# Isaac-McPadden/Farkle_II

Hardware: AMD Instinct MI355X
Metric: simulated games/sec (whole node) at k=2, fixed strategy-grid size (higher is better)
Workload: dtype int32; 1 GPU; BASELINE configs[1]: k=2, 64-strategy grid, 10^7 games per GPU per step, root_seed 42, counts-only tallies; k=2, root_seed=42, parallelism=shuffle-range split x1, device=AMD Radeon Graphics, arch=gfx950:sramecc+:xnack-, compute_units=256, clock_mhz=2400

## Files before the change

### farkle_ii_amd/csrc/farkle_hip.hip

```cpp
#include "fk_kernels.h"
#include "fk_shard_writer.h"
#include "fk_perm_wave.h"
#include "fk_row_columns_seats.h"
#include "fk_matchups.h"
#include "fk_game_stats.h"
#include "fk_bootstrap.h"

#include <dlfcn.h>
#include <rccl/rccl.h>
#include <unistd.h>

#include <algorithm>
#include <atomic>
#include <chrono>
#include <memory>
#include <mutex>
#include <sys/mman.h>
#include <unordered_map>
#include <thread>
#include <cstdarg>
#include <cstdio>
#include <cstring>
#include <string>
#include <vector>
// ... 16 lines not shown
    }
};

struct ChunkSet {
    DevBuf perm, draws, state, inc, seat_idx, order, classes, misc, pools;
    DevBuf blocks, game_block, game_row;
    hipEvent_t ready = nullptr;
    hipEvent_t ev[4] = {nullptr, nullptr, nullptr, nullptr};
    bool prepared = false;
    bool side = false;
    ChunkDesc desc;
    SeedArgs sa{};
};

struct GameStatsReq {
    int64_t rare_target;
    uint32_t rounds_bins, margin_bins;
    int64_t *s_counts, *s_rounds, *s_runner, *s_spread;
    int64_t *g_counts, *g_rounds, *g_runner;
    int64_t spill_capacity;
    int64_t *spill_count;
    int32_t *spill;
};

struct fk_ctx {
    int device = 0;
    hipStream_t stream = nullptr;
    hipStream_t prep_stream = nullptr;
    ChunkSet sets[2];
    int cur = 0;
    uint64_t table_epoch = 0;
    bool hint_valid = false;
    uint64_t hint_begin = 0, hint_end = 0;
    int32_t hint_state = 0, pipeline = 1;
    hipDeviceProp_t prop{};
    std::string err;
    fk_timing timing{};
    std::string play_instance;
    hipEvent_t ev[8] = {nullptr, nullptr, nullptr, nullptr, nullptr, nullptr, nullptr, nullptr};
    int32_t *err_host = nullptr;
    hipEvent_t main_idle = nullptr;
    struct PendingTimer {
        float *acc;
        hipEvent_t a, b;
    };
    std::vector<PendingTimer> pending;
// ... 18 lines not shown
    int32_t batch_threshold = 0;
    int32_t use_lds_tally = -1;
    int32_t block = 0;
    int32_t hc = -1;
    int32_t hc_waves = 5;
    int32_t hc_block = 256;
    int32_t hc_tables = 1;
    int32_t hc_inc_regs = 1;
    int32_t hc_cl = -1;
    DevBuf lds_tables;
    DevBuf cold;
    int32_t clock_stamps = 0;
    DevBuf clk;
    int clk_grid = 0;
    DevBuf lag_v, lag_out, lag_lags, lag_edge, lag_tmp;
    DevBuf m_ids, m_dig, m_seat, m_rnd;
    DevBuf mr[36];
    uint64_t matchup_sort_mask = ~0ull;
    DevBuf g_rec, g_out;
    int64_t game_stats_window = 0;
    const GameStatsReq *gstats = nullptr;
    DevBuf boot[8];
    int64_t bootstrap_block = 0;
    bool ran_hc = false;
    int32_t perm_split = -1;
    int32_t columns_by_seat = -1;
    int32_t perm_draw_wave = -1;
    void *comm = nullptr;
    int comm_rank = 0, comm_world = 1;
    bool comm_async = false;
    bool comm_lost = false;
    bool comm_timeout_set = false;
    int32_t comm_timeout_ms = 120000;
    DevBuf comm_buf;
    DevBuf rows_alt;
    const int32_t *columns_ids = nullptr;
    uint32_t *want_shuffle_seeds = nullptr, *want_game_seeds = nullptr;
    DevBuf ids;
    hipStream_t copy_stream = nullptr;
    hipEvent_t ev_rows[2] = {nullptr, nullptr}, ev_copy[2] = {nullptr, nullptr};
    int32_t rows_async = 0;
    hipEvent_t ev_call_copy[FK_ROWS_EVENTS] = {};
    uint32_t rows_calls = 0;
    uint8_t *mail = nullptr;
    size_t mail_cap = 0, mail_used = 0;
    struct Letter { void *dst; size_t off, bytes; };
    std::vector<Letter> letters;
    int32_t last_rows_event = -1;
    int64_t rows_chunk_games = 4000000;
// ... 144 lines not shown
    ss_begin(p, 2u , purpose, (uint32_t)root_seed, (uint32_t)(root_seed >> 32));
    ss_absorb64(p, k);
    return p;
}

struct LaunchPlan {
    int block = 0, grid = 0, cus = 1;
    mutable int launched_grid = 0;
    mutable const char *instance = nullptr;
    size_t lds = 0;
    bool lds_tally = false;
    bool lean = false;
    bool gs = false;
    bool blk = false;
    bool hc = false;
    bool hc_lt = false;
    int hc_ki = 0;
    bool hc_cl = false;
    int wpe = 4;
    uint32_t mixed_flags = 0xff00u;
};

constexpr size_t LDS_LIMIT = 160 * 1024;

size_t play_lds_bytes(int32_t k, int block, bool lean, bool gs, bool lds_tally, int32_t S, bool blocks_mode = false) {
    const size_t per_lane = (size_t)(lean ? LEAN_DW : NF) * 4 * (size_t)(gs ? 1 : k) + (blocks_mode ? 4 : 0);
    return per_lane * (size_t)block + (lds_tally ? (size_t)S * LT_COLS * 8 : 0);
}

LaunchPlan plan_play(const fk_ctx *c, int32_t k, int64_t S, bool single_batch, int32_t target_score, bool blocks_mode = false) {
    LaunchPlan best;
    const bool lean_ok = ceil_div50(target_score) <= LEAN_MAX_TARGET50;
    if (blocks_mode) {
        if (!lean_ok) return best;
        best.block = 768;
        best.lean = true;
        best.blk = true;
        best.wpe = 6;
        best.lds = play_lds_bytes(2, 768, true, false, false, 0, true);
        const int per_cu = c->blocks_per_cu > 0 ? std::min(2, c->blocks_per_cu) : 2;
        best.grid = c->prop.multiProcessorCount * per_cu;
        best.cus = c->prop.multiProcessorCount;
        return best;
    }
    const bool want_tally = single_batch && !blocks_mode && (c->use_lds_tally != 0) && S <= 4096;
    int best_lanes = -1;
// ... 297 lines not shown
            const uint32_t n_words = (uint32_t)(bytes / 4);
            hipLaunchKernelGGL(fk_mail_kernel, dim3(std::min<uint32_t>((n_words + 255u) / 256u, 1024u)), dim3(256), 0, c->stream,
                               static_cast<const uint32_t *>(src), reinterpret_cast<uint32_t *>(c->mail + off), n_words);
            HIPCHK(c, hipGetLastError());
            c->letters.push_back({dst, off, bytes});
            c->mail_used = off + bytes;
            return FK_OK;
        }
    }
    HIPCHK(c, hipMemcpyAsync(dst, src, bytes, hipMemcpyDeviceToHost, c->stream));
    return FK_OK;
}

void reserve_mail(fk_ctx *c, size_t bytes) {
    if (!c->letters.empty() || bytes <= c->mail_cap || !rows_dma_pending(c)) return;
    if (c->mail) (void)hipHostFree(c->mail);
    c->mail = nullptr;
    c->mail_cap = 0;
    const size_t cap = std::max<size_t>((size_t)4 << 20, (bytes + ((size_t)1 << 20)) & ~(((size_t)1 << 20) - 1));
    if (hipHostMalloc(reinterpret_cast<void **>(&c->mail), cap, hipHostMallocDefault) == hipSuccess) c->mail_cap = cap;
    else (void)hipGetLastError();
}

void deliver_mail(fk_ctx *c) {
    for (const auto &l : c->letters) std::memcpy(l.dst, c->mail + l.off, l.bytes);
    c->letters.clear();
    c->mail_used = 0;
}

int check_device_error(fk_ctx *c, const int32_t *d_err, int64_t game_base, const char *what) {
    int32_t h[2] = {0, 0};
    const int rc = post_d2h(c, h, d_err, sizeof(h));
    if (rc) return rc;
    HIPCHK(c, hipStreamSynchronize(c->stream));
    deliver_mail(c);
    return report_device_error(c, h, game_base, what);
}

int upload_overrides(fk_ctx *c, std::vector<DevOverride> &dov) {
    if (dov.empty()) return FK_OK;
    std::sort(dov.begin(), dov.end(), [](const DevOverride &x, const DevOverride &y) { return x.game < y.game; });
    int rc = ensure(c, c->ov, dov.size() * sizeof(DevOverride));
    if (rc) return rc;
    HIPCHK(c, hipMemcpyAsync(c->ov.p, dov.data(), dov.size() * sizeof(DevOverride), hipMemcpyHostToDevice, c->stream));
    HIPCHK(c, hipStreamSynchronize(c->stream));
    return FK_OK;
}


int seed_stage(fk_ctx *c, int si, hipStream_t st, SeedArgs &sa, bool full_state, bool timed) {
    ChunkSet &cs = c->sets[si];
    sa.state_dw = full_state ? STATE_DW : 4u;
    int rc = ensure(c, cs.state, (size_t)sa.n_games * sa.k * sa.state_dw * 4);
    if (rc) return rc;
    rc = ensure(c, cs.inc, (size_t)sa.n_games * sa.k * 16);
    if (rc) return rc;
    rc = ensure(c, cs.misc, 512);
    if (rc) return rc;
    HIPCHK(c, hipMemsetAsync(cs.misc.p, 0, 512, st));
    sa.state = static_cast<uint32_t *>(cs.state.p);
    sa.inc = static_cast<uint4 *>(cs.inc.p);
    sa.seat_idx = nullptr;
    if (sa.perm_T && !full_state) {
        rc = ensure(c, cs.seat_idx, (size_t)sa.n_games * sa.k * 2);
        if (rc) return rc;
        sa.seat_idx = static_cast<uint16_t *>(cs.seat_idx.p);
    }
    if (sa.blocks) {
        hipLaunchKernelGGL(fk_block_map_kernel, dim3((sa.n_games + 255u) / 256u), dim3(256), 0, st, sa.blocks, sa.n_blocks,
                           sa.n_games, const_cast<uint32_t *>(sa.game_block), const_cast<uint32_t *>(sa.game_row));
        HIPCHK(c, hipGetLastError());
    }
    if ((sa.perm_T || sa.blocks) && c->longest_first) {
        rc = ensure(c, cs.order, (size_t)sa.n_games * 4);
        if (rc) return rc;
        sa.sched = static_cast<uint32_t *>(cs.order.p);
        sa.sched_ctr = reinterpret_cast<uint32_t *>(static_cast<uint8_t *>(cs.misc.p) + 256);
        rc = ensure(c, cs.classes, 64);
        if (rc) return rc;
        HIPCHK(c, hipMemsetAsync(cs.classes.p, 0, 64, st));
        sa.class_ctr = static_cast<const uint32_t *>(cs.classes.p);
        sa.patience = static_cast<const uint8_t *>(c->slow.p);
    } else {
        sa.sched = nullptr;
    }
    if (timed) (void)hipEventRecord(cs.ev[2], st);
    sa.pools = nullptr;
    if (!sa.coords) {
        const uint32_t n = sa.blocks ? sa.n_blocks : (sa.gps ? (sa.n_games + sa.gps - 1u) / sa.gps : 1u);
        rc = ensure(c, cs.pools, (size_t)n * 16);
        if (rc) return rc;
        sa.pools = static_cast<const uint4 *>(cs.pools.p);
        hipLaunchKernelGGL(fk_pool_kernel, dim3((n + 255u) / 256u), dim3(256), 0, st, sa.prefix, sa.shuffle0, sa.pair, sa.order, sa.blocks, n,
                           static_cast<uint4 *>(cs.pools.p));
    }
    if (sa.sched)
        hipLaunchKernelGGL(fk_class_count_kernel, dim3(std::min<uint32_t>((sa.n_games + SEED_BLOCK - 1u) / SEED_BLOCK, 1024u)), dim3(SEED_BLOCK), 0,
                           st, sa.perm_T, sa.perm_slots, sa.S, sa.k, sa.n_sh, sa.n_games, sa.patience,
                           sa.blocks ? sa.game_row : nullptr, static_cast<uint32_t *>(cs.classes.p));
    hipLaunchKernelGGL(fk_seed_kernel, dim3((sa.n_games + SEED_BLOCK - 1u) / SEED_BLOCK), dim3(SEED_BLOCK), 0, st, sa);
    if (timed) (void)hipEventRecord(cs.ev[3], st);
    HIPCHK(c, hipGetLastError());
    return FK_OK;
}

size_t game_workspace_bytes(int32_t k, bool full_state, bool recs, bool rows) {
    return (size_t)k * ((full_state ? STATE_DW * 4 : 18) + 16) + 8 + (recs ? REC_DW * 4 + 4 : 0) +
           (rows ? sizeof(fk_row_hdr) + sizeof(fk_seat) * (size_t)k : 0);
}

int launch_play_stage(fk_ctx *c, const SeedArgs &sa, PlayArgs &pa, const LaunchPlan &plan, bool want_state, bool want_rec0, bool want_recs) {
    ChunkSet &cs = CSET(c);
    int rc;
    if (want_rec0) {
        rc = ensure(c, c->rec0, (size_t)sa.n_games * 4);
        if (rc) return rc;
    }
    if (want_recs) {
        rc = ensure(c, c->recs, (size_t)sa.n_games * REC_DW * 4);
// ... 79 lines not shown

int finish_play(fk_ctx *c, const PlayArgs &pa, int64_t game_base, const char *what) {
    const int rc_dev = check_device_error(c, pa.err, game_base, what);
    const int rc = finish_timers(c);
    return rc_dev ? rc_dev : rc;
}

int run_chunk(fk_ctx *c, const SeedArgs &sa_in, PlayArgs pa, const LaunchPlan &plan, bool want_state, bool want_rec0, bool want_recs,
              int64_t game_base, const char *what) {
    SeedArgs sa = sa_in;
    ChunkSet &cs = CSET(c);
    cs.prepared = false;
    cs.side = false;
    HIPCHK(c, hipStreamWaitEvent(c->stream, cs.ready, 0));
    (void)hipEventRecord(cs.ev[0], c->stream);
    (void)hipEventRecord(cs.ev[1], c->stream);
    int rc = seed_stage(c, c->cur, c->stream, sa, plan.gs || want_state, true);
    if (rc) return rc;
    rc = launch_play_stage(c, sa, pa, plan, want_state, want_rec0, want_recs);
    if (rc) return rc;
    return finish_play(c, pa, game_base, what);
}

int prep_tournament_chunk(fk_ctx *c, int si, hipStream_t st_seed, const ChunkDesc &d, SeedArgs &sa) {
    ChunkSet &cs = c->sets[si];
    cs.prepared = false;
    hipStream_t st = c->stream;
    HIPCHK(c, hipStreamWaitEvent(st, cs.ready, 0));
    const int32_t S = (int32_t)d.S;
    const uint32_t n_sh = d.n_sh, slots = d.slots, gps = d.S / d.k;
    const uint32_t perm_blocks = (n_sh + slots - 1u) / slots;
    const SeedPool perm_prefix = seed_prefix(101u , d.root, (uint64_t)d.k);
    int rc = ensure(c, cs.perm, (size_t)perm_blocks * S * slots * 2);
    if (rc) return rc;
    (void)hipEventRecord(cs.ev[0], st);
    {
        const size_t perm_lds = (size_t)slots * S * 2;
        static int perm_configured = -1;
        if (perm_configured != c->device) {
            HIPCHK(c, hipFuncSetAttribute(reinterpret_cast<const void *>(&fk_perm_kernel),
                                          hipFuncAttributeMaxDynamicSharedMemorySize, (int)LDS_LIMIT));
            HIPCHK(c, hipFuncSetAttribute(reinterpret_cast<const void *>(&fk_perm_apply_kernel),
                                          hipFuncAttributeMaxDynamicSharedMemorySize, (int)LDS_LIMIT));
            HIPCHK(c, hipFuncSetAttribute(reinterpret_cast<const void *>(&fk_perm_parallel_kernel),
                                          hipFuncAttributeMaxDynamicSharedMemorySize, (int)(LDS_LIMIT - 1024)));
            perm_configured = c->device;
        }
        const bool split = c->perm_split >= 1 || (c->perm_split < 0 && S >= 1024 && n_sh >= 256);
        const size_t pp_lds = (size_t)S * 14;
        const bool parallel = split && c->perm_split != 1 && pp_lds <= LDS_LIMIT - 1024;
        const bool wave_draw = c->perm_draw_wave == 1 || (c->perm_draw_wave < 0 && n_sh <= WAVE_DRAW_MAX_SH);
        if (parallel) {
            const uint32_t groups = ((uint32_t)S - 1u + 7u) / 8u, row_u4 = groups + 1u;
            rc = ensure(c, cs.draws, (size_t)n_sh * row_u4 * 16);
            if (rc) return rc;
            if (wave_draw)
                hipLaunchKernelGGL(fk_perm_draw_wave_kernel, dim3((n_sh + WAVE_DRAW_BLOCK / 64 - 1u) / (WAVE_DRAW_BLOCK / 64)), dim3(WAVE_DRAW_BLOCK), 0, st,
                                   perm_prefix, d.sh0, n_sh, (uint32_t)S, 1u, row_u4, static_cast<uint4 *>(cs.draws.p));
            else
                hipLaunchKernelGGL(fk_perm_draw_kernel, dim3((n_sh + DRAW_BLOCK - 1u) / DRAW_BLOCK), dim3(DRAW_BLOCK), 0, st,
                                   perm_prefix, d.sh0, n_sh, (uint32_t)S, 1u, row_u4, static_cast<uint4 *>(cs.draws.p));
            hipLaunchKernelGGL(fk_perm_parallel_kernel, dim3(n_sh), dim3(PP_BLOCK), pp_lds, st,
                               static_cast<uint4 *>(cs.draws.p), row_u4, n_sh, (uint32_t)S);
            hipLaunchKernelGGL(fk_perm_block_kernel, dim3(((uint32_t)S + 255u) / 256u, perm_blocks), dim3(256), 0, st,
                               static_cast<const uint16_t *>(cs.draws.p), row_u4 * 8u, n_sh, (uint32_t)S, slots,
                               static_cast<uint16_t *>(cs.perm.p));
        } else if (split) {
            const uint32_t n_sh_pad = (n_sh + 63u) & ~63u, groups = ((uint32_t)S - 1u + 7u) / 8u;
            rc = ensure(c, cs.draws, (size_t)groups * n_sh_pad * 16);
            if (rc) return rc;
            if (wave_draw)
                hipLaunchKernelGGL(fk_perm_draw_wave_kernel, dim3((n_sh + WAVE_DRAW_BLOCK / 64 - 1u) / (WAVE_DRAW_BLOCK / 64)), dim3(WAVE_DRAW_BLOCK), 0, st,
                                   perm_prefix, d.sh0, n_sh, (uint32_t)S, n_sh_pad, 1u, static_cast<uint4 *>(cs.draws.p));
            else
                hipLaunchKernelGGL(fk_perm_draw_kernel, dim3((n_sh + DRAW_BLOCK - 1u) / DRAW_BLOCK), dim3(DRAW_BLOCK), 0, st,
                                   perm_prefix, d.sh0, n_sh, (uint32_t)S, n_sh_pad, 1u, static_cast<uint4 *>(cs.draws.p));
            hipLaunchKernelGGL(fk_perm_apply_kernel, dim3(perm_blocks), dim3(PERM_BLOCK), perm_lds, st,
                               static_cast<const uint4 *>(cs.draws.p), n_sh_pad, n_sh, (uint32_t)S, slots,
                               static_cast<uint16_t *>(cs.perm.p));
        } else {
            hipLaunchKernelGGL(fk_perm_kernel, dim3(perm_blocks), dim3(PERM_BLOCK), perm_lds, st,
                               perm_prefix, d.sh0, n_sh, (uint32_t)S, slots, static_cast<uint16_t *>(cs.perm.p));
        }
        HIPCHK(c, hipGetLastError());
    }
    (void)hipEventRecord(cs.ev[1], st);
    sa = SeedArgs{};
    sa.prefix = seed_prefix(103u , d.root, (uint64_t)d.k);
    sa.coords = nullptr;
    sa.shuffle0 = d.sh0;
    sa.gps = gps;
    sa.k = d.k;
    sa.n_games = n_sh * gps;
    sa.perm_T = static_cast<const uint16_t *>(cs.perm.p);
    sa.perm_slots = slots;
    sa.S = d.S;
    sa.n_sh = n_sh;
    if (st_seed != st) {
        HIPCHK(c, hipStreamWaitEvent(st_seed, cs.ev[1], 0));
        HIPCHK(c, hipStreamWaitEvent(st_seed, c->main_idle, 0));
    }
    rc = seed_stage(c, si, st_seed, sa, d.state_dw == STATE_DW, true);
    if (rc) return rc;
    HIPCHK(c, hipEventRecord(cs.ready, st_seed));
    cs.desc = d;
    cs.prepared = true;
    cs.side = (st_seed == c->prep_stream);
    return FK_OK;
}

int rows_pass(fk_ctx *c, const SeedArgs &sa, bool scheduled, uint32_t n_games, uint32_t gps, uint32_t n_sh, bool perm_mode, uint8_t *d_rows) {
    const uint32_t *inv = scheduled ? static_cast<const uint32_t *>(c->inv.p) : nullptr;
    const uint32_t row_dw = 1u + 7u * sa.k;
    uint32_t block = 256;
    while (block > 64 && (size_t)block * row_dw * 4 > 65536) block -= 64;
    const size_t tile = (size_t)block * row_dw * 4;
    if (tile <= 65536) {
        static int configured = -1;
        if (configured != c->device) {
            HIPCHK(c, hipFuncSetAttribute(reinterpret_cast<const void *>(&fk_rows_kernel<true>), hipFuncAttributeMaxDynamicSharedMemorySize, 65536));
            configured = c->device;
        }
        hipLaunchKernelGGL(fk_rows_kernel<true>, dim3((n_games + block - 1u) / block), dim3(block), tile, c->stream,
                           static_cast<const uint32_t *>(CSET(c).state.p), static_cast<const uint32_t *>(c->recs.p), inv, n_games, gps, n_sh,
                           sa.k, perm_mode ? 1u : 0u, d_rows);
// ... 331 lines not shown
            (void)hipGetLastError();
            break;
        }
        c->hog.push_back(p);
    }
    if (free_now) *free_now = (int64_t)free_b;
    if (total) *total = (int64_t)total_b;
    return FK_OK;
}

static int32_t effective_comm_timeout_ms(const fk_ctx *c);

int fk_get_option(fk_ctx *c, const char *name, int64_t *value) {
    if (!c || !name || !value) return FK_ERR_ARG;
    const std::string n(name);
    if (n == "chunk_bytes") *value = c->chunk_bytes;
    else if (n == "workspace_percent") *value = c->workspace_percent;
    else if (n == "last_budget") *value = c->last_budget;
    else if (n == "oom_replays") *value = c->oom_replays;
    else if (n == "comm_timeout_ms") *value = effective_comm_timeout_ms(c);
    else if (n == "rows_chunk_games") *value = c->rows_chunk_games;
    else if (n == "rows_async") *value = c->rows_async;
    else if (n == "rows_event") *value = c->last_rows_event;
    else return fail(c, FK_ERR_ARG, "fk_get_option: unknown option %s", name);
    return FK_OK;
}

int fk_set_option(fk_ctx *c, const char *name, int64_t value) {
    if (!c || !name) return FK_ERR_ARG;
    std::string n(name);
    if (n == "chunk_bytes") c->chunk_bytes = std::max<int64_t>(value, 1 << 20);
    else if (n == "workspace_percent") c->workspace_percent = (int32_t)std::min<int64_t>(std::max<int64_t>(value, 1), 100000);
    else if (n == "comm_timeout_ms") {
        c->comm_timeout_ms = (int32_t)std::min<int64_t>(std::max<int64_t>(value, 0), 86400000);
        c->comm_timeout_set = true;
    }
    else if (n == "batch_threshold") c->batch_threshold = (int32_t)value;
    else if (n == "use_lds_tally") c->use_lds_tally = (int32_t)value;
    else if (n == "longest_first") c->longest_first = (int32_t)value;
    else if (n == "blocks_per_cu") c->blocks_per_cu = (int32_t)value;
    else if (n == "max_waves") c->max_waves = (int32_t)std::min<int64_t>(std::max<int64_t>(value, 1), 8);
    else if (n == "lean") c->lean = (int32_t)value;
    else if (n == "state_store") c->gs = (int32_t)value;
    else if (n == "rows_chunk_games") c->rows_chunk_games = std::max<int64_t>(value, 1);
    else if (n == "rows_async") c->rows_async = value != 0;
    else if (n == "resident_tally") {
        c->resident = value != 0;
        c->acc_n = 0;
    } else if (n == "hot_cold") {
        if (value != -1 && value != 0) return fail(c, FK_ERR_ARG, "hot_cold is -1 (auto: four and more seats) or 0 (never)");
        c->hc = (int32_t)value;
    }
    else if (n == "clock_stamps") c->clock_stamps = value != 0;
    else if (n == "perm_split") c->perm_split = (int32_t)value;
    else if (n == "perm_draw_wave") c->perm_draw_wave = (int32_t)value;
    else if (n == "columns_by_seat") c->columns_by_seat = (int32_t)value;
    else if (n == "pipeline") c->pipeline = (int32_t)value;
    else if (n == "uniform_flags") c->uniform_flags_opt = (int32_t)value;
    else if (n == "matchup_sort_key_mask") c->matchup_sort_mask = (uint64_t)value;
    else if (n == "game_stats_window") c->game_stats_window = std::max<int64_t>(value, 0);
    else if (n == "bootstrap_block") c->bootstrap_block = std::max<int64_t>(value, 0);
    else if (n == "block") {
        if (value != 0 && value != 64 && value != 128 && value != 256 && value != 512 && value != 768 && value != 1024)
            return fail(c, FK_ERR_ARG, "block must be 0, 64, 128, 256, 512, 768 (lean records only) or 1024");
        c->block = (int32_t)value;
    } else return fail(c, FK_ERR_ARG, "unknown option %s", name);
    return FK_OK;
}

int fk_tournament_run(fk_ctx *c, const fk_strategy *strategies, int32_t S, int32_t k, uint64_t root_seed,
                      uint64_t shuffle_begin, uint64_t shuffle_end, uint32_t shuffles_per_batch, int32_t target_score,
                      int32_t max_rounds, const fk_override *ov, int32_t n_ov, int64_t *tally, void *rows, int32_t *perms) {
    return fk_tournament_run_stats(c, strategies, S, k, root_seed, shuffle_begin, shuffle_end, shuffles_per_batch, target_score,
                                   max_rounds, ov, n_ov, tally, rows, perms, nullptr);
}

int fk_tournament_run_columns(fk_ctx *c, const fk_strategy *strategies, int32_t S, int32_t k, uint64_t root_seed, uint64_t shuffle_begin,
                              uint64_t shuffle_end, uint32_t shuffles_per_batch, int32_t target_score, int32_t max_rounds,
// ... 484 lines not shown
    if (lag && lag->m_digest) {
        if ((rc = ensure(c, c->m_ids, sizeof(int32_t) * (size_t)S))) return rc;
        if ((rc = ensure(c, c->m_dig, (size_t)chunk_sh * gps * 8))) return rc;
        if ((rc = ensure(c, c->m_seat, (size_t)chunk_sh * gps * 2 * (size_t)k))) return rc;
        if ((rc = ensure(c, c->m_rnd, (size_t)chunk_sh * gps * 2))) return rc;
        HIPCHK(c, hipMemcpyAsync(c->m_ids.p, lag->ids, sizeof(int32_t) * (size_t)S, hipMemcpyHostToDevice, c->stream));
    }

    const uint32_t g_rb = gst ? gst->rounds_bins : 0u, g_mb = gst ? gst->margin_bins : 0u;
    const uint32_t g_wr = c->game_stats_window > 0 ? (uint32_t)std::min<int64_t>(g_rb, c->game_stats_window) : g_rb;
    const uint32_t g_wm = c->game_stats_window > 0 ? (uint32_t)std::min<int64_t>(g_mb, c->game_stats_window) : g_mb;
    const size_t g_sc = 0, g_sr = g_sc + (size_t)S * fkg::N_COUNTS, g_sru = g_sr + (size_t)S * g_rb, g_ssp = g_sru + (size_t)S * g_mb,
                 g_gc = g_ssp + (size_t)S * g_mb, g_gr = g_gc + fkg::N_COUNTS, g_gru = g_gr + g_rb, g_cnt = g_gru + g_mb, g_u64 = g_cnt + 1;
    fkg::Spill g_spill{};
    if (gst) {
        if ((rc = ensure(c, c->g_rec, (size_t)chunk_sh * gps * 16))) return rc;
        if ((rc = ensure(c, c->g_out, g_u64 * 8 + (size_t)std::max<int64_t>(gst->spill_capacity, 1) * 12))) return rc;
        HIPCHK(c, hipMemsetAsync(c->g_out.p, 0, g_u64 * 8, c->stream));
        g_spill.count = static_cast<unsigned long long *>(c->g_out.p) + g_cnt;
        g_spill.entries = reinterpret_cast<int32_t *>(static_cast<unsigned long long *>(c->g_out.p) + g_u64);
        g_spill.cap = (uint64_t)gst->spill_capacity;
    }

    const uint32_t slots = (uint32_t)std::max<size_t>(1, std::min<size_t>(PERM_BLOCK, LDS_LIMIT / ((size_t)S * 2)));
    const uint32_t state_dw = (plan.gs || want_state) ? STATE_DW : 4u;
    auto describe = [&](uint64_t first_shuffle, uint32_t count, uint32_t dw) {
        ChunkDesc d;
        d.epoch = c->table_epoch;
        d.root = root_seed;
        d.sh0 = first_shuffle;
        d.n_sh = count;
        d.S = (uint32_t)S;
        d.k = (uint32_t)k;
        d.state_dw = dw;
        d.sched = c->longest_first ? 1u : 0u;
        d.slots = slots;
        return d;
    };
    const bool hinted = c->hint_valid && c->hint_end > c->hint_begin;
    const uint64_t hint_begin = c->hint_begin, hint_end = c->hint_end;
    const uint32_t hint_dw = (plan.gs || c->hint_state) ? STATE_DW : 4u;
    c->hint_valid = false;

    std::vector<uint16_t> perm_host;
    bool deferred = false;
    int64_t deferred_base = 0;
    for (uint64_t done = 0; done < n_sh_total; done += chunk_sh) {
        const uint32_t n_sh = (uint32_t)std::min<uint64_t>(chunk_sh, n_sh_total - done);
        const uint64_t sh0 = shuffle_begin + done;
        const uint32_t n_games = n_sh * gps;
        const uint32_t perm_blocks = (n_sh + slots - 1u) / slots;

        const ChunkDesc d = describe(sh0, n_sh, state_dw);
        int ready_set = -1;
        for (int si : {c->cur ^ 1, c->cur})
            if (c->sets[si].prepared && c->sets[si].desc == d) ready_set = si;
        bool wait_ready = false;
        if (ready_set >= 0) {
            c->cur = ready_set;
            wait_ready = true;
        } else {
            if (c->sets[c->cur].prepared) c->cur ^= 1;
            rc = prep_tournament_chunk(c, c->cur, c->stream, d, CSET(c).sa);
            if (rc) return rc;
        }
        CSET(c).prepared = false;
        const SeedArgs sa = CSET(c).sa;
        if (perms) {
            if (wait_ready) HIPCHK(c, hipStreamWaitEvent(c->stream, CSET(c).ready, 0));
            wait_ready = false;
            perm_host.resize((size_t)perm_blocks * S * slots);
            HIPCHK(c, hipMemcpyAsync(perm_host.data(), CSET(c).perm.p, perm_host.size() * 2, hipMemcpyDeviceToHost, c->stream));
            HIPCHK(c, hipStreamSynchronize(c->stream));
            for (uint32_t s = 0; s < n_sh; ++s)
                for (int32_t i = 0; i < S; ++i)
                    perms[(size_t)(done + s) * S + i] = perm_host[((size_t)(s / slots) * S + i) * slots + s % slots];
// ... 46 lines not shown
        pa.lds_tables = static_cast<const uint8_t *>(c->lds_tables.p);

        HIPCHK(c, hipEventRecord(c->main_idle, c->stream));
        if (c->pipeline) {
            ChunkDesc next{};
            bool have_next = false;
            if (done + chunk_sh < n_sh_total) {
                next = describe(sh0 + n_sh, (uint32_t)std::min<uint64_t>(chunk_sh, n_sh_total - done - chunk_sh), state_dw);
                have_next = true;
            } else if (hinted) {
                next = describe(hint_begin, (uint32_t)std::min<uint64_t>(chunk_sh, hint_end - hint_begin), hint_dw);
                have_next = true;
            }
            if (have_next) {
                rc = prep_tournament_chunk(c, c->cur ^ 1, c->prep_stream, next, c->sets[c->cur ^ 1].sa);
                if (rc) return rc;
            }
        }
        if (wait_ready) HIPCHK(c, hipStreamWaitEvent(c->stream, c->sets[c->cur].ready, 0));
        rc = launch_play_stage(c, sa, pa, plan, want_state, want_recs, want_recs);
        if (rc) return rc;
        const bool defer_check = done + chunk_sh >= n_sh_total && !rows && c->err_host;
        if (defer_check) {
            HIPCHK(c, hipMemcpyAsync(c->err_host, pa.err, 2 * sizeof(int32_t), hipMemcpyDeviceToHost, c->stream));
            deferred = true;
            deferred_base = (int64_t)done * gps;
        } else {
            rc = finish_play(c, pa, (int64_t)done * gps, "tournament");
            if (rc) return rc;
        }
        const bool scheduled = c->longest_first != 0;
        if (want_state && scheduled) {
            rc = ensure(c, c->inv, (size_t)n_games * 4);
            if (rc) return rc;
            hipLaunchKernelGGL(fk_invert_sched_kernel, dim3((n_games + 255u) / 256u), dim3(256), 0, c->stream,
                               static_cast<const uint32_t *>(CSET(c).order.p), n_games, static_cast<uint32_t *>(c->inv.p));
        }
        if (seat_stats || gst) {
            rc = ensure(c, CSET(c).draws, (size_t)perm_blocks * S * slots * 2);
            if (rc) return rc;
            const uint32_t cells = perm_blocks * (uint32_t)S * slots;
            hipLaunchKernelGGL(fk_invert_perm_kernel, dim3((cells + 255u) / 256u), dim3(256), 0, c->stream,
                               static_cast<const uint16_t *>(CSET(c).perm.p), (uint32_t)S, slots, n_sh, static_cast<uint16_t *>(CSET(c).draws.p));
        }
        if (gst) {
            unsigned long long *o = static_cast<unsigned long long *>(c->g_out.p);
            const uint32_t rec_grid = std::max<uint32_t>(1u, std::min<uint32_t>((n_games + 255u) / 256u, 2048u));
// ... 111 lines not shown
                                   static_cast<const uint32_t *>(CSET(c).state.p), static_cast<const uint32_t *>(c->recs.p),
                                   scheduled ? static_cast<const uint32_t *>(c->inv.p) : nullptr, n_games, gps, n_sh, (uint32_t)k, 1u,
                                   static_cast<const int32_t *>(c->ids.p), static_cast<uint8_t *>(row_buf.p), rows_per_shuffle);
                HIPCHK(c, hipGetLastError());
            } else {
                rc = rows_pass(c, sa, scheduled, n_games, gps, n_sh, true, static_cast<uint8_t *>(row_buf.p));
                if (rc) return rc;
            }
            HIPCHK(c, hipEventRecord(c->ev_rows[rb], c->stream));
            HIPCHK(c, hipStreamWaitEvent(c->copy_stream, c->ev_rows[rb], 0));
            HIPCHK(c, hipMemcpyAsync(static_cast<uint8_t *>(rows) + (size_t)done * rows_per_shuffle, row_buf.p,
                                     (size_t)n_sh * rows_per_shuffle, hipMemcpyDeviceToHost, c->copy_stream));
            HIPCHK(c, hipEventRecord(c->ev_copy[rb], c->copy_stream));
        }
    }
    if (rows && c->rows_async) {
        c->last_rows_event = (int32_t)(c->rows_calls % FK_ROWS_EVENTS);
        HIPCHK(c, hipEventRecord(c->ev_call_copy[c->last_rows_event], c->copy_stream));
        ++c->rows_calls;
    } else if (rows) {
        HIPCHK(c, hipStreamSynchronize(c->copy_stream));
    }
    const uint32_t n_rows = (uint32_t)(n_batches * (uint64_t)S);
    hipLaunchKernelGGL(fk_finalize_tally, dim3((n_rows + 255u) / 256u), dim3(256), 0, c->stream,
                       static_cast<unsigned long long *>(c->tally.p), n_rows, (uint32_t)S, shuffles_per_batch, n_sh_total, 1u);
    HIPCHK(c, hipGetLastError());
    c->last_tally_bytes = tally_bytes;
    HIPCHK(c, hipEventRecord(t1, c->stream));
    const size_t game_seed_bytes = c->want_game_seeds ? (size_t)n_sh_total * gps * 4 : 0, shuffle_seed_bytes = c->want_shuffle_seeds ? (size_t)n_sh_total * 4 : 0;
    reserve_mail(c, tally_bytes + game_seed_bytes + shuffle_seed_bytes + 256);
    rc = post_d2h(c, tally, c->tally.p, tally_bytes);
    if (rc) return rc;
    if (game_seed_bytes + shuffle_seed_bytes) {
        const size_t shuffle_at = (game_seed_bytes + 255u) & ~(size_t)255u;
        rc = ensure(c, c->dbg[5], shuffle_at + shuffle_seed_bytes);
        if (rc) return rc;
        uint8_t *d_seeds = static_cast<uint8_t *>(c->dbg[5].p);
        if (game_seed_bytes) {
            const size_t n = (size_t)n_sh_total * gps;
            hipLaunchKernelGGL(fk_game_seed_kernel, dim3((unsigned)((n + 255) / 256)), dim3(256), 0, c->stream, seed_prefix(102u , root_seed, (uint64_t)k),
                               shuffle_begin, (uint32_t)n_sh_total, gps, reinterpret_cast<uint32_t *>(d_seeds));
            HIPCHK(c, hipGetLastError());
            rc = post_d2h(c, c->want_game_seeds, d_seeds, game_seed_bytes);
            if (rc) return rc;
        }
        if (shuffle_seed_bytes) {
            hipLaunchKernelGGL(fk_game_seed_kernel, dim3((unsigned)((n_sh_total + 255) / 256)), dim3(256), 0, c->stream, seed_prefix(100u , root_seed, (uint64_t)k),
                               shuffle_begin, (uint32_t)n_sh_total, 1u, reinterpret_cast<uint32_t *>(d_seeds + shuffle_at));
            HIPCHK(c, hipGetLastError());
            rc = post_d2h(c, c->want_shuffle_seeds, d_seeds + shuffle_at, shuffle_seed_bytes);
            if (rc) return rc;
        }
    }
    if (seat_stats) HIPCHK(c, hipMemcpyAsync(seat_stats, c->stats.p, stats_bytes, hipMemcpyDeviceToHost, c->stream));
    if (seat_ratios) HIPCHK(c, hipMemcpyAsync(seat_ratios, c->ratios.p, ratio_bytes, hipMemcpyDeviceToHost, c->stream));
// ... 860 lines not shown
```

### farkle_ii_amd/csrc/fk_kernels.h

```cpp
#pragma once

#include "../../include/farkle_hip.h"
#include "fk_device.h"

#include <hip/hip_runtime.h>

using namespace fk;

namespace {

constexpr uint32_t HC_AFTER_6_WORDS = ss_hc(24);
constexpr uint32_t HC_AFTER_12_WORDS = ss_hc(48);
constexpr uint32_t HC_AFTER_14_WORDS = ss_hc(56);

enum : uint32_t { MODE_PERM = 0, MODE_LIST = 1, MODE_BLOCKS = 2 };

enum : uint32_t {
    F_LO0 = 0, F_LO1, F_HI0, F_HI1, F_INC_LO0, F_INC_LO1, F_INC_HI0, F_INC_HI1,
    F_BUF, F_SCORE, F_CA, F_CB, F_CC, F_CD, F_CE, F_SPX, F_SPY, NF
};
constexpr uint32_t CE_HAS_SCORED = 1u << 16, CE_HAS_BUF = 1u << 17;
constexpr uint32_t CE_IDX_SHIFT = 18;
constexpr uint32_t LEAN_DW = 10;
constexpr int32_t LEAN_MAX_TARGET50 = 64000;
// ... 442 lines not shown
    __shared__ uint32_t cnt[SCHED_CLASSES];
    if (threadIdx.x < SCHED_CLASSES) cnt[threadIdx.x] = 0u;
    __syncthreads();
    for (uint32_t base = blockIdx.x * blockDim.x; base < n_games; base += gridDim.x * blockDim.x) {
        const uint32_t t = base + threadIdx.x;
        uint32_t cls = SCHED_CLASSES;
        if (t < n_games) {
            if (game_block) {
                cls = schedule_class_block(patience, game_block[t]);
            } else {
                const uint32_t g_local = t / n_sh, sh_local = t - g_local * n_sh;
                cls = schedule_class(perm_T, perm_slots, S, k, patience, sh_local, g_local);
            }
        }
        for (uint32_t cidx = 0; cidx < SCHED_CLASSES; ++cidx) {
            const uint64_t m = __ballot(cls == cidx);
            if (m && lane_id() == 0u) atomicAdd(&cnt[cidx], (uint32_t)__popcll(m));
        }
    }
    __syncthreads();
    if (threadIdx.x < SCHED_CLASSES && cnt[threadIdx.x]) atomicAdd(&class_ctr[threadIdx.x], cnt[threadIdx.x]);
}

__global__ __launch_bounds__(SEED_BLOCK) void fk_seed_kernel(SeedArgs a) {
    __shared__ uint32_t wave_cnt[SCHED_CLASSES][SEED_BLOCK / 64];
    __shared__ uint32_t block_base[SCHED_CLASSES];
    const uint32_t t = blockIdx.x * blockDim.x + threadIdx.x;
    const bool valid = t < a.n_games;
    uint32_t id = t, sh_local = 0, g_local = t;
    if (a.perm_T) {
        g_local = t / a.n_sh;
        sh_local = t - g_local * a.n_sh;
        id = sh_local * a.gps + g_local;
    } else if (a.gps) {
        sh_local = t / a.gps;
        g_local = t - sh_local * a.gps;
    }
    uint32_t slot = t;
    if (a.sched) {
        uint32_t cls = SCHED_CLASSES;
        if (valid) cls = a.blocks ? schedule_class_block(a.patience, a.game_row[t])
                                  : schedule_class(a.perm_T, a.perm_slots, a.S, a.k, a.patience, sh_local, g_local);
        const uint32_t wave = threadIdx.x >> 6;
        uint64_t mine_m = 0;
        for (uint32_t cidx = 0; cidx < SCHED_CLASSES; ++cidx) {
            const uint64_t m = __ballot(cls == cidx);
// ... 83 lines not shown
        const size_t rec = (size_t)p_slot * a.k + s;
        uint4 *dst = reinterpret_cast<uint4 *>(a.state + rec * a.state_dw);
        dst[0] = make_uint4((uint32_t)r.lo, (uint32_t)(r.lo >> 32), (uint32_t)r.hi, (uint32_t)(r.hi >> 32));
        if (a.state_dw == STATE_DW) {
            uint32_t idx = s;
            if (a.perm_T) idx = perm_at(a.perm_T, a.S, a.perm_slots, p_sh, p_g * a.k + s);
            else if (a.seat_strategy) idx = (uint32_t)a.seat_strategy[(size_t)p_id * a.k + s];
            else if (a.blocks) idx = 2u * a.blocks[p_blk].row + s;
            dst[1] = make_uint4(0u, 0u, 0u, 0u);
            dst[2] = make_uint4(0u, 0u, 0u, idx);
        } else if (a.seat_idx && a.perm_T) {
            a.seat_idx[rec] = perm_at(a.perm_T, a.S, a.perm_slots, p_sh, p_g * a.k + s);
        }
        a.inc[rec] = make_uint4((uint32_t)r.inc_lo, (uint32_t)(r.inc_lo >> 32), (uint32_t)r.inc_hi, (uint32_t)(r.inc_hi >> 32));
    }
}

__global__ void fk_add_i64_kernel(unsigned long long *acc, const unsigned long long *src, size_t n) {
    const size_t i = (size_t)blockIdx.x * blockDim.x + threadIdx.x;
    if (i < n) acc[i] += src[i];
}

__global__ void fk_finalize_tally(unsigned long long *tally, uint32_t n_rows, uint32_t S, uint32_t spb, uint64_t n_sh_total,
                                  uint32_t derive_completed) {
    const uint32_t i = blockIdx.x * blockDim.x + threadIdx.x;
    if (i >= n_rows) return;
    unsigned long long *t = tally + (size_t)i * FK_TALLY_COLS;
    if (derive_completed) {
        const uint64_t batch = i / S, first = batch * spb;
        const uint64_t in_batch = first + spb <= n_sh_total ? spb : n_sh_total - first;
        t[1] = in_batch;
        t[2] = in_batch - t[3];
    } else {
        t[1] = t[2] + t[3];
    }
}

template <int BLOCK, bool LEAN, int WPE, uint32_t MIXED, bool GS, bool BLK = false, int KC = 0>
__global__ __launch_bounds__(BLOCK) __attribute__((amdgpu_waves_per_eu(WPE))) void fk_play_kernel(PlayArgs a) {
    static_assert(!GS || LEAN, "state-store instances stage the lean record");
    static_assert(!BLK || (LEAN && !GS), "block-index instances use lean LDS records");
    extern __shared__ __attribute__((aligned(16))) uint32_t lds[];
    const uint32_t tid = threadIdx.x;
    const uint32_t K = KC ? (uint32_t)KC : a.k;
    constexpr uint32_t NFIELDS = LEAN ? LEAN_DW : (uint32_t)NF;
    unsigned long long *tl = reinterpret_cast<unsigned long long *>(lds + NFIELDS * (GS ? 1u : K) * BLOCK);
    uint32_t *lane_block = lds + NFIELDS * (GS ? 1u : K) * BLOCK + tid;
    clock_stamp(a.clk, 0u);

    if (a.use_lds_tally) {
        for (uint32_t i = tid; i < a.S * LT_COLS; i += BLOCK) tl[i] = 0ull;
        __syncthreads();
    }

    enum : uint32_t { ST_FRESH = 0, ST_ACTIVE = 1, ST_ENDED = 2, ST_DONE = 3 };
    uint32_t st = ST_FRESH;
    uint32_t pool_next = 0, pool_end = 0, exhausted = 0;

// ... 1011 lines not shown
```

Before: 1.109 billion games/s.

## Add small-grid perm kernel with fused class counting and merged tally tail

For small strategy grids, a new perm kernel runs one shuffle per thread in an interleaved LDS layout, sized to the launch. When longest-first scheduling is on, it also counts schedule classes, so the separate class-count kernel and memset in the seed stage are skipped. The finalize-tally kernel now writes the tally and the error words straight into pinned host mail, which replaces separate D2H copies at the tail. The costs are an extra code path with new slot-sizing heuristics and device writes into host memory.

```diff
diff --git a/farkle_ii_amd/csrc/farkle_hip.hip b/farkle_ii_amd/csrc/farkle_hip.hip
--- a/farkle_ii_amd/csrc/farkle_hip.hip
+++ b/farkle_ii_amd/csrc/farkle_hip.hip
@@ -62,6 +62,16 @@
     int64_t *spill_count;
     int32_t *spill;
 };
+
+#ifndef FK_DEFAULT_PERM_SMALL_LAYOUT
+#define FK_DEFAULT_PERM_SMALL_LAYOUT 1
+#endif
+#ifndef FK_DEFAULT_FUSED_CLASS_COUNT
+#define FK_DEFAULT_FUSED_CLASS_COUNT 1
+#endif
+#ifndef FK_DEFAULT_MERGED_TAIL
+#define FK_DEFAULT_MERGED_TAIL 1
+#endif
 
 struct fk_ctx {
     int device = 0;
@@ -126,9 +136,13 @@
     const GameStatsReq *gstats = nullptr;
     DevBuf boot[8];
     int64_t bootstrap_block = 0;
+    int32_t last_perm_slots = 0;
     bool ran_hc = false;
     int32_t perm_split = -1;
     int32_t columns_by_seat = -1;
+    int32_t perm_small_layout = FK_DEFAULT_PERM_SMALL_LAYOUT;
+    int32_t merged_tail = FK_DEFAULT_MERGED_TAIL;
+    int32_t fused_class_count = FK_DEFAULT_FUSED_CLASS_COUNT;
     int32_t perm_draw_wave = -1;
     void *comm = nullptr;
     int comm_rank = 0, comm_world = 1;
@@ -319,6 +333,7 @@
 };
 
 constexpr size_t LDS_LIMIT = 160 * 1024;
+
 
 size_t play_lds_bytes(int32_t k, int block, bool lean, bool gs, bool lds_tally, int32_t S, bool blocks_mode = false) {
     const size_t per_lane = (size_t)(lean ? LEAN_DW : NF) * 4 * (size_t)(gs ? 1 : k) + (blocks_mode ? 4 : 0);
@@ -662,6 +677,18 @@
     else (void)hipGetLastError();
 }
 
+bool ensure_mail(fk_ctx *c, size_t bytes) {
+    if (bytes <= c->mail_cap) return true;
+    if (!c->letters.empty()) return false;
+    if (c->mail) (void)hipHostFree(c->mail);
+    c->mail = nullptr;
+    c->mail_cap = 0;
+    const size_t cap = std::max<size_t>((size_t)4 << 20, (bytes + ((size_t)1 << 20)) & ~(((size_t)1 << 20) - 1));
+    if (hipHostMalloc(reinterpret_cast<void **>(&c->mail), cap, hipHostMallocDefault) == hipSuccess) c->mail_cap = cap;
+    else (void)hipGetLastError();
+    return bytes <= c->mail_cap;
+}
+
 void deliver_mail(fk_ctx *c) {
     for (const auto &l : c->letters) std::memcpy(l.dst, c->mail + l.off, l.bytes);
     c->letters.clear();
@@ -688,7 +715,7 @@
 }
 
 
-int seed_stage(fk_ctx *c, int si, hipStream_t st, SeedArgs &sa, bool full_state, bool timed) {
+int seed_stage(fk_ctx *c, int si, hipStream_t st, SeedArgs &sa, bool full_state, bool timed, bool classes_sized = false) {
     ChunkSet &cs = c->sets[si];
     sa.state_dw = full_state ? STATE_DW : 4u;
     int rc = ensure(c, cs.state, (size_t)sa.n_games * sa.k * sa.state_dw * 4);
@@ -718,7 +745,7 @@
         sa.sched_ctr = reinterpret_cast<uint32_t *>(static_cast<uint8_t *>(cs.misc.p) + 256);
         rc = ensure(c, cs.classes, 64);
         if (rc) return rc;
-        HIPCHK(c, hipMemsetAsync(cs.classes.p, 0, 64, st));
+        if (!classes_sized) HIPCHK(c, hipMemsetAsync(cs.classes.p, 0, 64, st));
         sa.class_ctr = static_cast<const uint32_t *>(cs.classes.p);
         sa.patience = static_cast<const uint8_t *>(c->slow.p);
     } else {
@@ -734,7 +761,7 @@
         hipLaunchKernelGGL(fk_pool_kernel, dim3((n + 255u) / 256u), dim3(256), 0, st, sa.prefix, sa.shuffle0, sa.pair, sa.order, sa.blocks, n,
                            static_cast<uint4 *>(cs.pools.p));
     }
-    if (sa.sched)
+    if (sa.sched && !classes_sized)
         hipLaunchKernelGGL(fk_class_count_kernel, dim3(std::min<uint32_t>((sa.n_games + SEED_BLOCK - 1u) / SEED_BLOCK, 1024u)), dim3(SEED_BLOCK), 0,
                            st, sa.perm_T, sa.perm_slots, sa.S, sa.k, sa.n_sh, sa.n_games, sa.patience,
                            sa.blocks ? sa.game_row : nullptr, static_cast<uint32_t *>(cs.classes.p));
@@ -860,6 +887,34 @@
     return finish_play(c, pa, game_base, what);
 }
 
+bool perm_large_path(const fk_ctx *c, uint32_t S, uint32_t n_sh) {
+    return c->perm_split >= 1 || (c->perm_split < 0 && S >= 1024 && n_sh >= 256);
+}
+
+bool perm_small_path(const fk_ctx *c, uint32_t S, uint32_t n_sh) {
+    const uint32_t least = c->perm_small_layout > 1 ? (uint32_t)c->perm_small_layout : 64u;
+    return c->perm_small_layout != 0 && !perm_large_path(c, S, n_sh) && (size_t)least * S * 2 <= LDS_LIMIT;
+}
+
+uint32_t plan_perm_slots(const fk_ctx *c, uint32_t S, uint32_t n_sh) {
+    if (!perm_small_path(c, S, n_sh)) return (uint32_t)std::max<size_t>(1, std::min<size_t>(PERM_BLOCK, LDS_LIMIT / ((size_t)S * 2)));
+    if (c->perm_small_layout > 1) return (uint32_t)c->perm_small_layout;
+    const uint32_t cus = (uint32_t)std::max(c->prop.multiProcessorCount, 1);
+    uint32_t best = 64, best_places = 0;
+    for (uint32_t s = 64; s <= 512; s *= 2) {
+        const size_t lds = (size_t)s * S * 2;
+        if (lds > LDS_LIMIT) break;
+        const uint32_t per_cu = (uint32_t)std::min<size_t>(std::min<size_t>(LDS_LIMIT / lds, 32u / (s / 64u)), 16u);
+        const uint32_t places = per_cu * s * cus;
+        if (places >= n_sh) return s;
+        if (places > best_places) {
+            best = s;
+            best_places = places;
+        }
+    }
+    return best;
+}
+
 int prep_tournament_chunk(fk_ctx *c, int si, hipStream_t st_seed, const ChunkDesc &d, SeedArgs &sa) {
     ChunkSet &cs = c->sets[si];
     cs.prepared = false;
@@ -868,9 +923,17 @@
     const int32_t S = (int32_t)d.S;
     const uint32_t n_sh = d.n_sh, slots = d.slots, gps = d.S / d.k;
     const uint32_t perm_blocks = (n_sh + slots - 1u) / slots;
+    const bool small = perm_small_path(c, d.S, n_sh);
+    const bool fused = small && c->fused_class_count && c->longest_first;
+    c->last_perm_slots = (int32_t)slots;
     const SeedPool perm_prefix = seed_prefix(101u , d.root, (uint64_t)d.k);
     int rc = ensure(c, cs.perm, (size_t)perm_blocks * S * slots * 2);
     if (rc) return rc;
+    if (fused) {
+        rc = ensure(c, cs.classes, 64);
+        if (rc) return rc;
+        HIPCHK(c, hipMemsetAsync(cs.classes.p, 0, 64, st));
+    }
     (void)hipEventRecord(cs.ev[0], st);
     {
         const size_t perm_lds = (size_t)slots * S * 2;
@@ -878,13 +941,15 @@
         if (perm_configured != c->device) {
             HIPCHK(c, hipFuncSetAttribute(reinterpret_cast<const void *>(&fk_perm_kernel),
                                           hipFuncAttributeMaxDynamicSharedMemorySize, (int)LDS_LIMIT));
+            HIPCHK(c, hipFuncSetAttribute(reinterpret_cast<const void *>(&fk_perm_small_kernel),
+                                          hipFuncAttributeMaxDynamicSharedMemorySize, (int)LDS_LIMIT));
             HIPCHK(c, hipFuncSetAttribute(reinterpret_cast<const void *>(&fk_perm_apply_kernel),
                                           hipFuncAttributeMaxDynamicSharedMemorySize, (int)LDS_LIMIT));
             HIPCHK(c, hipFuncSetAttribute(reinterpret_cast<const void *>(&fk_perm_parallel_kernel),
                                           hipFuncAttributeMaxDynamicSharedMemorySize, (int)(LDS_LIMIT - 1024)));
             perm_configured = c->device;
         }
-        const bool split = c->perm_split >= 1 || (c->perm_split < 0 && S >= 1024 && n_sh >= 256);
+        const bool split = perm_large_path(c, d.S, n_sh);
         const size_t pp_lds = (size_t)S * 14;
         const bool parallel = split && c->perm_split != 1 && pp_lds <= LDS_LIMIT - 1024;
         const bool wave_draw = c->perm_draw_wave == 1 || (c->perm_draw_wave < 0 && n_sh <= WAVE_DRAW_MAX_SH);
@@ -916,6 +981,12 @@
             hipLaunchKernelGGL(fk_perm_apply_kernel, dim3(perm_blocks), dim3(PERM_BLOCK), perm_lds, st,
                                static_cast<const uint4 *>(cs.draws.p), n_sh_pad, n_sh, (uint32_t)S, slots,
                                static_cast<uint16_t *>(cs.perm.p));
+        } else if (small) {
+            uint32_t slots_log2 = 6;
+            while ((1u << slots_log2) < slots) ++slots_log2;
+            hipLaunchKernelGGL(fk_perm_small_kernel, dim3(perm_blocks), dim3(slots), perm_lds, st,
+                               perm_prefix, d.sh0, n_sh, (uint32_t)S, slots_log2, d.k, static_cast<const uint8_t *>(c->slow.p),
+                               fused ? static_cast<uint32_t *>(cs.classes.p) : nullptr, static_cast<uint16_t *>(cs.perm.p));
         } else {
             hipLaunchKernelGGL(fk_perm_kernel, dim3(perm_blocks), dim3(PERM_BLOCK), perm_lds, st,
                                perm_prefix, d.sh0, n_sh, (uint32_t)S, slots, static_cast<uint16_t *>(cs.perm.p));
@@ -938,7 +1009,7 @@
         HIPCHK(c, hipStreamWaitEvent(st_seed, cs.ev[1], 0));
         HIPCHK(c, hipStreamWaitEvent(st_seed, c->main_idle, 0));
     }
-    rc = seed_stage(c, si, st_seed, sa, d.state_dw == STATE_DW, true);
+    rc = seed_stage(c, si, st_seed, sa, d.state_dw == STATE_DW, true, fused);
     if (rc) return rc;
     HIPCHK(c, hipEventRecord(cs.ready, st_seed));
     cs.desc = d;
@@ -1316,6 +1387,10 @@
     else if (n == "rows_chunk_games") *value = c->rows_chunk_games;
     else if (n == "rows_async") *value = c->rows_async;
     else if (n == "rows_event") *value = c->last_rows_event;
+    else if (n == "perm_small_layout") *value = c->perm_small_layout;
+    else if (n == "fused_class_count") *value = c->fused_class_count;
+    else if (n == "merged_tail") *value = c->merged_tail;
+    else if (n == "last_perm_slots") *value = c->last_perm_slots;
     else return fail(c, FK_ERR_ARG, "fk_get_option: unknown option %s", name);
     return FK_OK;
 }
@@ -1348,6 +1423,12 @@
     else if (n == "clock_stamps") c->clock_stamps = value != 0;
     else if (n == "perm_split") c->perm_split = (int32_t)value;
     else if (n == "perm_draw_wave") c->perm_draw_wave = (int32_t)value;
+    else if (n == "perm_small_layout") {
+        if (value != 0 && value != 1 && value != 64 && value != 128 && value != 256 && value != 512)
+            return fail(c, FK_ERR_ARG, "perm_small_layout is 0, 1 (slots sized to the launch) or a forced slot count of 64, 128, 256 or 512");
+        c->perm_small_layout = (int32_t)value;
+    } else if (n == "fused_class_count") c->fused_class_count = value != 0;
+    else if (n == "merged_tail") c->merged_tail = value != 0;
     else if (n == "columns_by_seat") c->columns_by_seat = (int32_t)value;
     else if (n == "pipeline") c->pipeline = (int32_t)value;
     else if (n == "uniform_flags") c->uniform_flags_opt = (int32_t)value;
@@ -1878,7 +1959,6 @@
         g_spill.cap = (uint64_t)gst->spill_capacity;
     }
 
-    const uint32_t slots = (uint32_t)std::max<size_t>(1, std::min<size_t>(PERM_BLOCK, LDS_LIMIT / ((size_t)S * 2)));
     const uint32_t state_dw = (plan.gs || want_state) ? STATE_DW : 4u;
     auto describe = [&](uint64_t first_shuffle, uint32_t count, uint32_t dw) {
         ChunkDesc d;
@@ -1890,7 +1970,7 @@
         d.k = (uint32_t)k;
         d.state_dw = dw;
         d.sched = c->longest_first ? 1u : 0u;
-        d.slots = slots;
+        d.slots = plan_perm_slots(c, (uint32_t)S, count);
         return d;
     };
     const bool hinted = c->hint_valid && c->hint_end > c->hint_begin;
@@ -1898,6 +1978,9 @@
     const uint32_t hint_dw = (plan.gs || c->hint_state) ? STATE_DW : 4u;
     c->hint_valid = false;
 
+    const bool merged_tail = c->merged_tail && !rows && c->err_host && tally && tally_bytes <= ((size_t)1 << 20) &&
+                             ensure_mail(c, ((c->mail_used + 63u) & ~(size_t)63u) + tally_bytes + 64);
+    const int32_t *deferred_err = nullptr;
     std::vector<uint16_t> perm_host;
     bool deferred = false;
     int64_t deferred_base = 0;
@@ -1905,9 +1988,9 @@
         const uint32_t n_sh = (uint32_t)std::min<uint64_t>(chunk_sh, n_sh_total - done);
         const uint64_t sh0 = shuffle_begin + done;
         const uint32_t n_games = n_sh * gps;
-        const uint32_t perm_blocks = (n_sh + slots - 1u) / slots;
 
         const ChunkDesc d = describe(sh0, n_sh, state_dw);
+        const uint32_t slots = d.slots, perm_blocks = (n_sh + slots - 1u) / slots;
         int ready_set = -1;
         for (int si : {c->cur ^ 1, c->cur})
             if (c->sets[si].prepared && c->sets[si].desc == d) ready_set = si;
@@ -2000,7 +2083,8 @@
         if (rc) return rc;
         const bool defer_check = done + chunk_sh >= n_sh_total && !rows && c->err_host;
         if (defer_check) {
-            HIPCHK(c, hipMemcpyAsync(c->err_host, pa.err, 2 * sizeof(int32_t), hipMemcpyDeviceToHost, c->stream));
+            if (merged_tail) deferred_err = pa.err;
+            else HIPCHK(c, hipMemcpyAsync(c->err_host, pa.err, 2 * sizeof(int32_t), hipMemcpyDeviceToHost, c->stream));
             deferred = true;
             deferred_base = (int64_t)done * gps;
         } else {
@@ -2158,15 +2242,25 @@
         HIPCHK(c, hipStreamSynchronize(c->copy_stream));
     }
     const uint32_t n_rows = (uint32_t)(n_batches * (uint64_t)S);
+    const bool mailed = merged_tail && deferred_err;
+    const size_t mail_at = (c->mail_used + 63u) & ~(size_t)63u;
     hipLaunchKernelGGL(fk_finalize_tally, dim3((n_rows + 255u) / 256u), dim3(256), 0, c->stream,
-                       static_cast<unsigned long long *>(c->tally.p), n_rows, (uint32_t)S, shuffles_per_batch, n_sh_total, 1u);
+                       static_cast<unsigned long long *>(c->tally.p), n_rows, (uint32_t)S, shuffles_per_batch, n_sh_total, 1u, deferred_err,
+                       mailed ? reinterpret_cast<unsigned long long *>(c->mail + mail_at) : nullptr);
     HIPCHK(c, hipGetLastError());
+    if (mailed) {
+        c->letters.push_back({tally, mail_at, tally_bytes});
+        c->letters.push_back({c->err_host, mail_at + tally_bytes, 2 * sizeof(int32_t)});
+        c->mail_used = mail_at + tally_bytes + 2 * sizeof(int32_t);
+    }
     c->last_tally_bytes = tally_bytes;
     HIPCHK(c, hipEventRecord(t1, c->stream));
     const size_t game_seed_bytes = c->want_game_seeds ? (size_t)n_sh_total * gps * 4 : 0, shuffle_seed_bytes = c->want_shuffle_seeds ? (size_t)n_sh_total * 4 : 0;
     reserve_mail(c, tally_bytes + game_seed_bytes + shuffle_seed_bytes + 256);
-    rc = post_d2h(c, tally, c->tally.p, tally_bytes);
-    if (rc) return rc;
+    if (!mailed) {
+        rc = post_d2h(c, tally, c->tally.p, tally_bytes);
+        if (rc) return rc;
+    }
     if (game_seed_bytes + shuffle_seed_bytes) {
         const size_t shuffle_at = (game_seed_bytes + 255u) & ~(size_t)255u;
         rc = ensure(c, c->dbg[5], shuffle_at + shuffle_seed_bytes);
diff --git a/farkle_ii_amd/csrc/fk_kernels.h b/farkle_ii_amd/csrc/fk_kernels.h
--- a/farkle_ii_amd/csrc/fk_kernels.h
+++ b/farkle_ii_amd/csrc/fk_kernels.h
@@ -488,6 +488,81 @@
     if (threadIdx.x < SCHED_CLASSES && cnt[threadIdx.x]) atomicAdd(&class_ctr[threadIdx.x], cnt[threadIdx.x]);
 }
 
+__global__ __launch_bounds__(512) void fk_perm_small_kernel(SeedPool prefix, uint64_t shuffle0, uint32_t n_sh, uint32_t S,
+                                                            uint32_t slots_log2, uint32_t k, const uint8_t *patience,
+                                                            uint32_t *class_ctr, uint16_t *perm_T) {
+    extern __shared__ __align__(16) uint16_t perm_em_lds[];
+    const uint32_t slots = 1u << slots_log2, slot = threadIdx.x;
+    const uint32_t sh = blockIdx.x * slots + slot;
+    const bool valid = sh < n_sh;
+    uint16_t *a = perm_em_lds + slot;
+    for (uint32_t e = 0; e < S; ++e) a[e << slots_log2] = valid ? (uint16_t)e : (uint16_t)0;
+    Rng r{};
+    if (valid) {
+        SeedPool p = prefix;
+        p.hc = HC_AFTER_6_WORDS;
+        ss_absorb64(p, shuffle0 + sh);
+#pragma unroll
+        for (int w = 0; w < 5; ++w) ss_absorb64(p, 0);
+        uint32_t g8[8];
+        ss_generate<8>(p, g8);
+        pcg_seed(r, g8);
+    }
+    uint32_t i = valid ? S - 1u : 0u;
+    auto consume = [&](uint32_t w) {
+        if (i >= 1u) {
+            const uint32_t j = w & (0xffffffffu >> __clz((int)i));
+            if (j <= i) {
+                const uint16_t ai = a[i << slots_log2], aj = a[j << slots_log2];
+                a[i << slots_log2] = aj;
+                a[j << slots_log2] = ai;
+                i -= 1u;
+            }
+        }
+    };
+    while (__ballot(i >= 1u)) {
+        const uint64_t o = pcg_next64(r);
+        consume((uint32_t)o);
+        consume((uint32_t)(o >> 32));
+    }
+    uint64_t c4[4] = {0, 0, 0, 0};
+    if (class_ctr) {
+        if (valid) {
+            const uint32_t gps = S / k;
+            for (uint32_t g = 0; g < gps; ++g) {
+                uint32_t sum = 0, n_never = 0;
+                for (uint32_t s = 0; s < k; ++s) {
+                    const uint32_t p = patience[a[(g * k + s) << slots_log2]];
+                    sum += p;
+                    n_never += (p == 3u) ? 1u : 0u;
+                }
+                const uint32_t cls = class_of(sum, n_never, k);
+                const uint64_t one = 1ull << ((cls & 3u) * 16u);
+#pragma unroll
+                for (uint32_t q = 0; q < 4; ++q) c4[q] += (cls >> 2) == q ? one : 0ull;
+            }
+        }
+    }
+    __syncthreads();
+    const uint4 *src = reinterpret_cast<const uint4 *>(perm_em_lds);
+    uint4 *out = reinterpret_cast<uint4 *>(perm_T + ((size_t)blockIdx.x * S << slots_log2));
+    for (uint32_t idx = threadIdx.x; idx < (S << slots_log2) / 8u; idx += slots) out[idx] = src[idx];
+    if (class_ctr) {
+        uint32_t *cnt = reinterpret_cast<uint32_t *>(perm_em_lds);
+        __syncthreads();
+        if (threadIdx.x < SCHED_CLASSES) cnt[threadIdx.x] = 0u;
+        __syncthreads();
+#pragma unroll
+        for (uint32_t cidx = 0; cidx < SCHED_CLASSES; ++cidx) {
+            uint32_t v = (uint32_t)(c4[cidx >> 2] >> ((cidx & 3u) * 16u)) & 0xffffu;
+            for (int d = 32; d >= 1; d >>= 1) v += __shfl_xor(v, d);
+            if (lane_id() == 0u && v) atomicAdd(&cnt[cidx], v);
+        }
+        __syncthreads();
+        if (threadIdx.x < SCHED_CLASSES && cnt[threadIdx.x]) atomicAdd(&class_ctr[threadIdx.x], cnt[threadIdx.x]);
+    }
+}
+
 __global__ __launch_bounds__(SEED_BLOCK) void fk_seed_kernel(SeedArgs a) {
     __shared__ uint32_t wave_cnt[SCHED_CLASSES][SEED_BLOCK / 64];
     __shared__ uint32_t block_base[SCHED_CLASSES];
@@ -617,8 +692,13 @@
 }
 
 __global__ void fk_finalize_tally(unsigned long long *tally, uint32_t n_rows, uint32_t S, uint32_t spb, uint64_t n_sh_total,
-                                  uint32_t derive_completed) {
+                                  uint32_t derive_completed, const int32_t *err, unsigned long long *mail) {
     const uint32_t i = blockIdx.x * blockDim.x + threadIdx.x;
+    if (mail && i == 0u) {
+        int32_t *e = reinterpret_cast<int32_t *>(mail + (size_t)n_rows * FK_TALLY_COLS);
+        e[0] = err[0];
+        e[1] = err[1];
+    }
     if (i >= n_rows) return;
     unsigned long long *t = tally + (size_t)i * FK_TALLY_COLS;
     if (derive_completed) {
@@ -629,6 +709,8 @@
     } else {
         t[1] = t[2] + t[3];
     }
+    if (mail)
+        for (uint32_t col = 0; col < FK_TALLY_COLS; ++col) mail[(size_t)i * FK_TALLY_COLS + col] = t[col];
 }
 
 template <int BLOCK, bool LEAN, int WPE, uint32_t MIXED, bool GS, bool BLK = false, int KC = 0>
```

Result: slower. 1.085 billion games/s (-2.2%).
